# sun-huangqingbo/multiplexed-image-annotator

Hardware: AMD Instinct MI355X
Metric: cells/sec annotated (whole node) (higher is better)
Workload: dtype f16

## Files before the change

### multiplexed-image-annotator_amd/_lib.py

```python
from __future__ import annotations

import ctypes
import os
from ctypes import POINTER, c_char_p, c_double, c_float, c_int32, c_int64, c_uint32, c_uint64, c_void_p

HERE = os.path.dirname(os.path.abspath(__file__))
LIB_PATH = os.path.join(HERE, "libribca_hip.so")
if os.environ.get("RIBCA_LIB"):
    LIB_PATH = os.environ["RIBCA_LIB"] if os.path.isabs(os.environ["RIBCA_LIB"]) else os.path.join(HERE, os.environ["RIBCA_LIB"])

TEST_LIB_PATH = LIB_PATH[:-3] + "_test.so"

_lib = None
_test_lib = None

SIGNATURES = {
    "ribca_version": (c_int32, []),
    "ribca_last_error": (c_char_p, []),
    "ribca_mask_minmax": (c_int32, [c_void_p, c_int64, c_void_p, c_void_p]),
    "ribca_label_table": (c_int32, [c_void_p, c_int32, c_int32, c_int32, c_void_p, c_void_p, c_void_p]),
    "ribca_channel_min": (c_int32, [c_void_p, c_int32, c_int64, c_void_p, c_void_p]),
    "ribca_extract_patches": (c_int32, [c_void_p, c_int32, c_int32, c_int32, c_void_p, c_void_p, c_void_p, c_void_p, c_void_p, c_int32,
                                        c_void_p, c_void_p, c_void_p]),
    "ribca_extract_patches_scaled": (c_int32, [c_void_p, c_int32, c_int32, c_int32, c_void_p, c_void_p, c_void_p, c_void_p, c_void_p, c_int32,
# ... 100 lines not shown
    "ribca_test_mx_weight_bytes": (c_int64, [c_int32, c_int32, c_int32]),
    "ribca_test_mx_pack_act": (c_int32, [c_void_p, c_int32, c_int32, c_int32, c_void_p, c_void_p, c_void_p, c_void_p]),
    "ribca_test_gemm_mx_resid": (c_int32, [c_void_p, c_int32, c_void_p, c_int32, c_int32, c_int32, c_int32, c_void_p, c_void_p, c_void_p, c_void_p,
                                           c_void_p, c_void_p, c_void_p, c_int32, c_void_p, c_void_p, c_void_p, c_void_p]),
    "ribca_test_gemm_mx_resid_packed": (c_int32, [c_void_p, c_void_p, c_void_p, c_int32, c_void_p, c_void_p, c_int32, c_int32, c_void_p, c_void_p, c_int32,
                                                  c_void_p, c_void_p, c_void_p, c_void_p]),
    "ribca_test_gemm_gelu_mx": (c_int32, [c_void_p, c_int32, c_void_p, c_int32, c_int32, c_int32, c_int32, c_void_p, c_void_p, c_void_p, c_void_p,
                                          c_void_p, c_void_p, c_void_p, c_void_p]),
    "ribca_test_gemm_mx_fc1": (c_int32, [c_void_p, c_int32, c_void_p, c_int32, c_int32, c_int32, c_int32, c_void_p, c_void_p, c_void_p, c_void_p,
                                         c_void_p, c_void_p, c_void_p, c_void_p, c_void_p, c_void_p, c_void_p, c_void_p]),
    "ribca_test_qkv_attention_mx": (c_int32, [c_void_p, c_int32, c_void_p, c_int32, c_int32, c_int32, c_int32, c_void_p, c_void_p, c_void_p, c_void_p,
                                              c_void_p, c_void_p, c_void_p, c_void_p, c_void_p, c_void_p, c_void_p, c_void_p, c_int32, c_void_p]),
    "ribca_test_gemm_resid_zmx": (c_int32, [c_int32, c_void_p, c_int32, c_void_p, c_int32, c_int32, c_int32, c_int32, c_void_p, c_void_p, c_void_p,
                                            c_void_p, c_void_p, c_void_p, c_void_p, c_int32, c_void_p, c_void_p, c_void_p, c_void_p, c_void_p,
                                            c_void_p, c_int32, c_void_p]),
    "ribca_test_gemm_fold": (c_int32, [c_int32, c_void_p, c_int32, c_void_p, c_int32, c_int32, c_int32, c_int32, c_void_p, c_void_p,
                                       c_void_p, c_void_p, c_int32, c_void_p]),
    "ribca_test_qkv_attention_fold": (c_int32, [c_void_p, c_int32, c_void_p, c_int32, c_int32, c_int32, c_int32, c_void_p, c_void_p,
                                                c_void_p, c_void_p, c_void_p, c_void_p, c_void_p, c_int32, c_void_p]),
    "ribca_test_gemm_duo_gelu": (c_int32, [c_void_p, c_int32, c_void_p, c_int32, c_int32, c_int32, c_int32, c_void_p, c_void_p, c_void_p,
                                           c_void_p, c_void_p, c_int32, c_void_p]),
    "ribca_test_cell_attention": (c_int32, [c_void_p, c_int32, c_void_p, c_int32, c_int32, c_int32, c_void_p, c_void_p, c_void_p, c_void_p, c_int32,
                                            c_void_p]),
    "ribca_gemm_padded_n": (c_int32, [c_int32]),
}


class RibcaError(RuntimeError):
    pass


class _Library:

    def __init__(self, handle):
        self._handle = handle

    def __getattr__(self, name):
        if name in SIGNATURES:
            fn = getattr(self._handle, name)
        elif name in TEST_SIGNATURES:
            fn = getattr(_load_test_lib(), name)
        else:
            raise AttributeError(f"{name} is declared neither in include/ribca_hip.h nor in include/ribca_hip_test.h")
        setattr(self, name, fn)
        return fn

# ... 61 lines not shown
```

### multiplexed-image-annotator_amd/build.py

```python
from __future__ import annotations

import concurrent.futures
import os
import subprocess
import sys

HERE = os.path.dirname(os.path.abspath(__file__))
CSRC = os.path.join(HERE, "csrc")
LIB = os.path.join(HERE, "libribca_hip.so")
LIB_TEST = os.path.join(HERE, "libribca_hip_test.so")
TEST_SOURCES = ["ribca_test_api.hip"]
EXPORTS = os.path.join(CSRC, "exports.map")
SOURCES = ["gemm_split16.hip", "gemm_duo.hip", "gemm_mx.hip", "attention.hip", "cell_attention.hip", "vit_misc.hip", "preprocess.hip", "preprocess_scaled.hip", "vote.hip", "colorize.hip", "knn.hip", "umap.hip", "hdbscan.hip", "regions.hip", "spectral.hip", "scatter.hip", "celltype_stats.hip", "enrichment.hip", "autocorr.hip", "local_autocorr.hip", "cooccurrence.hip", "normalize.hip", "ribca_api.hip"]
HEADERS = ["ribca_common.h", "ribca_kernels.h", "ribca_scratch.h", "ribca_perm.h", "ribca_status.h", "ribca_internal.h", "gemm_epi.h", os.path.join("..", "..", "include", "ribca_hip.h"),
           os.path.join("..", "..", "include", "ribca_hip_test.h")]
FLAGS = ["-O3", "--offload-arch=gfx950", "-fPIC", "-std=c++17", "-Wall", "-Wno-unused-function", "-fvisibility=hidden", "-fvisibility-inlines-hidden",
         "-fno-slp-vectorize"]


def source_fingerprint() -> str:
    import hashlib
    h = hashlib.sha256()
    for name in sorted(SOURCES + TEST_SOURCES) + sorted(HEADERS):
        path = os.path.normpath(os.path.join(CSRC, name))
        h.update(os.path.basename(path).encode() + b"\0")
        with open(path, "rb") as f:
            h.update(f.read())
    h.update(" ".join(FLAGS).encode())
    return h.hexdigest()


def _hipcc() -> str:
    for cand in (os.environ.get("HIPCC"), "/opt/rocm/bin/hipcc", "hipcc"):
        if cand and (os.path.isabs(cand) and os.path.exists(cand) or not os.path.isabs(cand)):
            return cand
    raise RuntimeError("hipcc not found")
# ... 52 lines not shown
```

### multiplexed-image-annotator_amd/csrc/ribca_api.hip

```cpp
#include <hip/hip_runtime.h>

#include <cmath>
#include <cstdarg>
#include <cstdlib>
#include <cstdio>
#include <cstring>
#include <string>
#include <vector>

#include "../../include/ribca_hip.h"
#include "ribca_common.h"
#include "ribca_internal.h"
#include "ribca_kernels.h"
#include "ribca_scratch.h"
#include "ribca_status.h"

using namespace ribca;

namespace {

int fail(const std::string& msg) { return api_fail(msg.c_str()); }
int hip_fail(hipError_t e, const char* what) { return api_hip_fail(e, what); }

inline int round_up(int v, int m) { return (v + m - 1) / m * m; }
// ... 57 lines not shown
}
int api_hip_fail(hipError_t e, const char* what) { return api_fail((std::string(what) + ": " + hipGetErrorString(e)).c_str()); }
int api_finish() {
  if (!g_launch_err.empty()) {
    const std::string m = g_launch_err;
    (void)hipGetLastError();
    return api_fail(m.c_str());
  }
  const hipError_t e = hipGetLastError();
  return e == hipSuccess ? 0 : api_hip_fail(e, "kernel launch");
}
const char* api_last_error() { return g_err.c_str(); }
}

struct BlockW {
  const float *ln1w, *ln1b, *qkvb, *projb, *ln2w, *ln2b, *fc1b, *fc2b;
  const uint16_t *qkvw, *projw, *fc1w, *fc2w;
  const uint16_t* qkvwf = nullptr;
  const uint16_t* fc1wf;
  const uint16_t *projwf = nullptr, *fc2wf = nullptr;
  const float *qkvc = nullptr, *qkvb2 = nullptr, *fc1c = nullptr, *fc1b2 = nullptr;
  const uint16_t* fc2mxh = nullptr; const unsigned char* fc2mxx = nullptr;
  const uint16_t *qkvmxh = nullptr, *fc1mxh = nullptr; const unsigned char *qkvmxx = nullptr, *fc1mxx = nullptr;
};

bool env_on(const char* name) { return !(getenv(name) && atoi(getenv(name)) == 0); }
struct Switches { bool mx, mxz, cell_attn; };
const Switches& switches() {
  static const Switches sw = {env_on("RIBCA_MX"), env_on("RIBCA_MXZ"), env_on("RIBCA_CELL_ATTN")};
  return sw;
}
bool mx_on(int D) { return switches().mx && (4 * D) % 128 == 0 && gemm_mx_supported(D, 4 * D); }
bool mx_z_on(int D) { return switches().mxz && mx_on(D) && D % 192 == 0; }

struct BlockPath {
  bool fold, mx_fc2, mx_z, cell_attn;
  BlockPath precise() const { return {fold, false, false, cell_attn}; }
  bool qkv_mx3() const { return mx_z && !cell_attn; }
};
BlockPath block_path(const AttnGeom& a, bool fold) {
  return {fold, fold && mx_on(a.D), fold && mx_z_on(a.D), fold && switches().cell_attn && cell_attention_supported(a.D, a.H, a.T)};
}

struct ribca_vit {
  int D, C, K, depth, Dp;
  BlockPath path;
  char* arena = nullptr;
  size_t arena_bytes = 0;
  const float *cls, *pos, *pe_b, *norm_w, *norm_b, *head_w, *head_b;
  const float* pe_w;
  std::vector<BlockW> layers;
};

struct ribca_mae {
  int L, enc_depth, dec_depth;
  BlockPath enc_path, dec_path;
  char* arena = nullptr;
  size_t arena_bytes = 0;
  const float *cls, *pos, *pe_b, *norm_w, *norm_b, *de_b, *mask_tok, *dpos, *dnorm_w, *dnorm_b, *pred_b;
  const uint16_t *pe_w, *de_w, *pred_w;
  std::vector<BlockW> enc, dec;
};

namespace {
// ... 7 lines not shown
    L.fc1c = c.take<float>(4 * D); L.fc1b2 = c.take<float>(4 * D);
  }
  L.ln1w = c.take<float>(D); L.ln1b = c.take<float>(D);
  L.qkvb = c.take<float>(3 * D); L.projb = c.take<float>(D);
  L.ln2w = c.take<float>(D); L.ln2b = c.take<float>(D);
  L.fc1b = c.take<float>(4 * D); L.fc2b = c.take<float>(D);
  L.qkvw = c.take<uint16_t>((size_t)gemm_padded_n(3 * D) * 2 * Dp);
  if (p.fold) L.qkvwf = c.take<uint16_t>((size_t)gemm_padded_n(3 * D) * 2 * Dp);
  L.projw = c.take<uint16_t>((size_t)gemm_padded_n(D) * 2 * Dp);
  if (p.fold) L.projwf = c.take<uint16_t>((size_t)gemm_padded_n(D) * 2 * Dp);
  L.fc1w = c.take<uint16_t>((size_t)gemm_padded_n(4 * D) * 2 * Dp);
  L.fc1wf = c.take<uint16_t>((size_t)gemm_padded_n(4 * D) * 2 * Dp);
  L.fc2w = c.take<uint16_t>((size_t)gemm_padded_n(D) * 2 * H4);
  if (p.fold) L.fc2wf = c.take<uint16_t>((size_t)gemm_padded_n(D) * 2 * H4);
  if (p.mx_fc2) {
    L.fc2mxh = c.take<uint16_t>(mx_wh_bytes(round_up(D, 16), H4) / 2);
    L.fc2mxx = c.take<unsigned char>(mx_wx_bytes(round_up(D, 16), H4));
  }
  if (p.mx_z) {
    const int Kz = round_up(D, 128);
    L.qkvmxh = c.take<uint16_t>(mx_wh_bytes(3 * D, Kz) / 2); L.qkvmxx = c.take<unsigned char>(mx_wx_bytes(3 * D, Kz));
    L.fc1mxh = c.take<uint16_t>(mx_wh_bytes(4 * D, Kz) / 2); L.fc1mxx = c.take<unsigned char>(mx_wx_bytes(4 * D, Kz));
  }
}

size_t layout(ribca_vit* m, char* base) {
  Carver c(base);
  const int D = m->D;
  m->cls = c.take<float>(D);
  m->pos = c.take<float>((size_t)kTokens * D);
  m->pe_b = c.take<float>(D);
  m->pe_w = c.take<float>((size_t)D * 16 * m->C);
  m->layers.resize(m->depth);
  for (auto& L : m->layers) layout_block(c, L, D, m->path);
  m->norm_w = c.take<float>(D); m->norm_b = c.take<float>(D);
  m->head_w = c.take<float>((size_t)m->K * D); m->head_b = c.take<float>(m->K);
  return c.off;
}

size_t layout_mae(ribca_mae* m, char* base) {
  Carver c(base);
  m->cls = c.take<float>(kEncD);
  m->pos = c.take<float>((size_t)(m->L + 1) * kEncD);
  m->pe_w = c.take<uint16_t>((size_t)gemm_padded_n(kEncD) * 2 * kTokPix);
  m->pe_b = c.take<float>(kEncD);
  m->enc.resize(m->enc_depth);
// ... 30 lines not shown
  void block(const BlockW& L, int D, const BlockPath& path) {
    const int Dp = round_up(D, 32);
    copy(L.ln1w, D); copy(L.ln1b, D);
    if (path.fold) {
      pack_fold(L.qkvw, 3 * D, D, Dp, L.ln1w, L.ln1b, L.qkvc, L.qkvb2);
      launch_pack_wf(L.qkvw, 2 * Dp, gemm_padded_n(3 * D), Dp, const_cast<uint16_t*>(L.qkvwf), s);
    } else pack(L.qkvw, 3 * D, D, Dp);
    copy(L.qkvb, 3 * D);
    pack(L.projw, D, D, Dp); copy(L.projb, D);
    if (path.fold) launch_pack_wf(L.projw, 2 * Dp, gemm_padded_n(D), Dp, const_cast<uint16_t*>(L.projwf), s);
    copy(L.ln2w, D); copy(L.ln2b, D);
    if (path.fold) pack_fold(L.fc1w, 4 * D, D, Dp, L.ln2w, L.ln2b, L.fc1c, L.fc1b2);
    else pack(L.fc1w, 4 * D, D, Dp);
    copy(L.fc1b, 4 * D);
    launch_pack_wf(L.fc1w, 2 * Dp, gemm_padded_n(4 * D), Dp, const_cast<uint16_t*>(L.fc1wf), s);
    pack(L.fc2w, D, 4 * D, 4 * D); copy(L.fc2b, D);
    if (path.fold) launch_pack_wf(L.fc2w, 2 * 4 * D, gemm_padded_n(D), 4 * D, const_cast<uint16_t*>(L.fc2wf), s);
    if (path.mx_fc2) launch_mx_pack_w(L.fc2w, 2 * 4 * D, round_up(D, 16), 4 * D, 4 * D, const_cast<uint16_t*>(L.fc2mxh), const_cast<unsigned char*>(L.fc2mxx), s);
    if (path.mx_z) {
      const int Kz = round_up(D, 128);
      launch_mx_pack_w(L.qkvw, 2 * Dp, 3 * D, Dp, Kz, const_cast<uint16_t*>(L.qkvmxh), const_cast<unsigned char*>(L.qkvmxx), s);
      launch_mx_pack_w(L.fc1w, 2 * Dp, 4 * D, Dp, Kz, const_cast<uint16_t*>(L.fc1mxh), const_cast<unsigned char*>(L.fc1mxx), s);
    }
  }
};
int64_t block_params(int64_t d) { return 2 * d + 3 * d * d + 3 * d + d * d + d + 2 * d + 4 * d * d + 4 * d + 4 * d * d + d; }

struct BlockWs {
  float* z; uint16_t* xa; uint16_t* q; uint16_t* k; uint16_t* vt; uint16_t* h;
  size_t qk_bytes, vt_bytes, xa_bytes;
  uint16_t* zps = nullptr; float2* part = nullptr; float2* rs = nullptr;
  MxAct zmx = MxAct{nullptr, nullptr, nullptr, 0, 0};
  size_t zmx_rows = 0;
};
BlockWs carve_blocks(Carver& c, int cells, const AttnGeom& a, const BlockPath& p) {
  BlockWs w;
  const size_t Mc = (size_t)cells * a.T;
  const int Dp = round_up(a.D, 32);
  if (p.fold) {
    w.z = nullptr;
    w.zps = c.take<uint16_t>(Mc * 2 * Dp);
    w.part = c.take<float2>(Mc * gemm_resid_part_rows(a.D));
    w.rs = c.take<float2>(Mc);
    if (p.mx_z) {
      const int Kz = round_up(a.D, 128);
      w.zmx.hi = c.take<uint16_t>(Mc * Kz);
      w.zmx.l8 = c.take<unsigned char>(Mc * Kz);
      w.zmx.sc = c.take<unsigned char>(Mc * (Kz / 32));
      w.zmx.Kp = Kz;
      w.zmx_rows = Mc;
    }
  } else {
    w.z = c.take<float>(Mc * a.D);
  }
  w.xa_bytes = Mc * 2 * Dp * sizeof(uint16_t);
  w.xa = c.take<uint16_t>(Mc * 2 * Dp);
  const size_t qk = (size_t)cells * a.H * a.TP * 2 * a.hdq;
  w.qk_bytes = qk * sizeof(uint16_t);
  w.q = c.take<uint16_t>(qk);
  w.k = c.take<uint16_t>(qk);
  const size_t vt = attention_v_elems(a, cells);
  w.vt_bytes = vt * sizeof(uint16_t);
  w.vt = c.take<uint16_t>(vt);
  w.h = c.take<uint16_t>(Mc * 2 * 4 * a.D);
  return w;
}
int zero_pads(const BlockWs& w, const BlockPath& p, hipStream_t s) {
  HIP_TRY(hipMemsetAsync(w.xa, 0, w.xa_bytes, s));
  if (p.fold) HIP_TRY(hipMemsetAsync(w.zps, 0, w.xa_bytes, s));
  HIP_TRY(hipMemsetAsync(w.q, 0, w.qk_bytes, s));
  HIP_TRY(hipMemsetAsync(w.k, 0, w.qk_bytes, s));
  HIP_TRY(hipMemsetAsync(w.vt, 0, w.vt_bytes, s));
  if (p.mx_z) {
    HIP_TRY(hipMemsetAsync(w.zmx.hi, 0, w.zmx_rows * w.zmx.Kp * 2, s));
    HIP_TRY(hipMemsetAsync(w.zmx.l8, 0, w.zmx_rows * w.zmx.Kp, s));
    HIP_TRY(hipMemsetAsync(w.zmx.sc, 0, w.zmx_rows * (w.zmx.Kp / 32), s));
  }
  return 0;
}
void run_block(const BlockW& L, const BlockWs& w, int cells, const AttnGeom& a, hipStream_t s) {
  const int D = a.D, Dp = round_up(D, 32), ld_x = 2 * Dp, ld_h = 2 * 4 * D, Mc = cells * a.T;
  const float scale = 1.0f / sqrtf((float)a.hd);
  { ProfScope ps(P_LN, s); launch_layernorm_ps(w.z, D, L.ln1w, L.ln1b, w.xa, ld_x, Mc, D, s); }
  {
    ProfScope ps(P_QKV, s);
    GemmArgs g{w.xa, ld_x, L.qkvw, ld_x, Mc, 3 * D, Dp, L.qkvb};
    launch_gemm_qkv(g, w.q, w.k, w.vt, a, scale, s);
// ... 20 lines not shown
void resid_ps_and_stats(const GemmArgs& g, const BlockWs& w, int ldz_rows, int D, bool want_stats, int prev_stride, hipStream_t s) {
  const ResidStatGeom sg = launch_gemm_resid_ps(g, w.zps, ldz_rows, want_stats ? w.part : nullptr, w.rs, prev_stride, s);
  if (want_stats) launch_ln_finalize(w.part, sg.tiles, g.M, sg.bn, D, w.rs, s);
}
void run_block_fold(const BlockW& L, const BlockWs& w, int cells, const AttnGeom& a, const BlockPath& p, bool next_mx3, hipStream_t s) {
  const int D = a.D, Dp = round_up(D, 32), ld_x = 2 * Dp, ld_h = 2 * 4 * D, Mc = cells * a.T;
  const float scale = 1.0f / sqrtf((float)a.hd);
  MxAct zmx = w.zmx;
  zmx.M = Mc;
  if (p.cell_attn) {
    ProfScope ps(P_CELL, s);
    launch_cell_qkv_attention(w.zps, ld_x, L.qkvw, ld_x, L.qkvb2, L.qkvc, w.rs, w.xa, ld_x, cells, D, scale, s);
  } else {
    {
      ProfScope ps(P_QKV, s);
      if (p.mx_z) {
        launch_gemm_mx_qkv_ln(zmx, MxWeight{L.qkvmxh, L.qkvmxx}, Mc, 3 * D, L.qkvb2, w.rs, L.qkvc, w.q, w.k, w.vt, a, scale, s);
      } else {
        GemmArgs g{w.zps, ld_x, L.qkvw, ld_x, Mc, 3 * D, Dp, L.qkvb2, L.qkvwf};
        launch_gemm_qkv_ln(g, w.rs, L.qkvc, w.q, w.k, w.vt, a, scale, s);
      }
    }
    { ProfScope ps(P_ATTN, s); launch_attention(w.q, w.k, w.vt, w.xa, ld_x, cells, a, s); }
  }
  {
    ProfScope ps(P_PROJ, s);
    GemmArgs g{w.xa, ld_x, L.projw, ld_x, Mc, D, Dp, L.projb, L.projwf};
    if (p.mx_z) {
      const ResidStatGeom sg = launch_gemm_resid_ps(g, w.zps, ld_x, w.part, w.rs, 1, s, false, &zmx);
      launch_ln_finalize(w.part, sg.tiles, Mc, sg.bn, D, w.rs, s);
    } else {
      resid_ps_and_stats(g, w, ld_x, D, true, 1, s);
    }
  }
  if (p.mx_fc2) {
    const size_t hn = (size_t)Mc * 4 * D;
    const MxAct hmx{w.h, reinterpret_cast<unsigned char*>(w.h + hn), reinterpret_cast<unsigned char*>(w.h + hn) + hn, 4 * D, Mc};
    {
      ProfScope ps(P_FC1, s);
      if (p.mx_z) {
        launch_gemm_mx_gelu(zmx, MxWeight{L.fc1mxh, L.fc1mxx}, Mc, 4 * D, L.fc1b2, w.rs, L.fc1c, hmx, s);
      } else {
        GemmArgs g{w.zps, ld_x, L.fc1w, ld_x, Mc, 4 * D, Dp, L.fc1b2, L.fc1wf};
        (void)launch_gemm_gelu_mx(g, w.rs, L.fc1c, hmx, s);
      }
    }
// ... 555 lines not shown
```

### multiplexed-image-annotator_amd/csrc/ribca_internal.h

```cpp
#pragma once
#include <stdint.h>

#include "ribca_kernels.h"
#include "ribca_status.h"

#define RIBCA_INTERNAL_VERSION 6002

#define RIBCA_INTERNAL_FUNCS(X)                                                                                                              \
  X(api_finish) X(api_fail) X(mx_wh_bytes) X(mx_wx_bytes) X(gemm_padded_n) X(gemm_resid_bn) X(gemm_resid_tiles) X(gemm_resid_part_rows)      \
  X(gemm_mx_supported) X(cell_attention_supported) X(make_attn_geom) X(launch_pack_wf)                                                      \
  X(launch_pack_weight) X(launch_pack_weight_fold) X(launch_mx_pack_w) X(launch_mx_pack_act) X(launch_layernorm_ps) X(launch_row_stats_ps)   \
  X(launch_ln_finalize) X(launch_gemm_resid) X(launch_gemm_gelu) X(launch_gemm_qkv) X(launch_gemm_qkv_ln) X(launch_gemm_gelu_ln)             \
  X(launch_gemm_gelu_mx) X(launch_gemm_resid_ps) X(launch_gemm_mx_resid) X(launch_gemm_mx_qkv_ln) X(launch_gemm_mx_gelu) X(launch_attention) \
  X(launch_cell_qkv_attention)

namespace ribca {
struct InternalTable {
  int32_t version;
  int32_t n_funcs;
#define RIBCA_X(name) decltype(&ribca::name) name;
  RIBCA_INTERNAL_FUNCS(RIBCA_X)
#undef RIBCA_X
};
}
```

### multiplexed-image-annotator_amd/csrc/ribca_kernels.h

```cpp
#pragma once
#include <hip/hip_runtime.h>
#include <stdint.h>

namespace ribca {

int gemm_pick_bn(int N);
int gemm_padded_n(int N);

struct GemmArgs {
  const uint16_t* A; int lda;
  const uint16_t* W; int ldw;
  int M, N, Kp;
  const float* bias;
  const uint16_t* WF = nullptr;
};
void launch_pack_wf(const uint16_t* W, int ldw, int Np, int Kp, uint16_t* WF, hipStream_t s);
void launch_gemm_resid(const GemmArgs& g, float* z, int ldz, hipStream_t s);
void launch_gemm_gelu(const GemmArgs& g, uint16_t* out, int ldo, hipStream_t s);
struct ResidStatGeom { int tiles, bn; };
struct MxAct { uint16_t* hi; unsigned char* l8; unsigned char* sc; int Kp; int M; };
ResidStatGeom launch_gemm_resid_ps(const GemmArgs& g, uint16_t* z, int ldz, float2* part, const float2* prev, int prev_stride, hipStream_t s,
                                   bool force_duo = false, const MxAct* zmx = nullptr);
int gemm_resid_tiles(int N);
int gemm_resid_bn(int N);
// ... 13 lines not shown
                        int dst_per_cell, hipStream_t s);

struct MxWeight { const uint16_t* wh; const unsigned char* wx; };
size_t mx_wh_bytes(int Np, int Kp);
size_t mx_wx_bytes(int Np, int Kp);
inline size_t mx_act_hi_elems(size_t M, int Kp128) { return M * (size_t)Kp128; }
void launch_mx_pack_w(const uint16_t* W, int ldw, int Np, int Ksrc, int Kp, uint16_t* WH, unsigned char* WX, hipStream_t s);
void launch_mx_pack_act(const uint16_t* ps, int ldps, int M, int Kp, const MxAct& a, hipStream_t s);
bool gemm_mx_supported(int N, int Kp);
bool launch_gemm_gelu_mx(const GemmArgs& g, const float2* rowstat, const float* csum, const MxAct& out, hipStream_t s);
ResidStatGeom launch_gemm_mx_resid(const MxAct& A, const MxWeight& W, int M, int N, const float* bias, uint16_t* z, int ldz, float2* part,
                                   const float2* prev, int prev_stride, hipStream_t s, const MxAct* zmx = nullptr);
void launch_gemm_mx_qkv_ln(const MxAct& A, const MxWeight& W, int M, int N, const float* bias, const float2* rowstat, const float* csum, uint16_t* q,
                           uint16_t* k, uint16_t* vt, const AttnGeom& a, float scale, hipStream_t s);
void launch_gemm_mx_gelu(const MxAct& A, const MxWeight& W, int M, int N, const float* bias, const float2* rowstat, const float* csum, const MxAct& out,
                         hipStream_t s);

void launch_attention(const uint16_t* q, const uint16_t* k, const uint16_t* vt, uint16_t* out, int ldo, int cells, const AttnGeom& a,
                      hipStream_t s, int q_tiles = 0);

bool cell_attention_supported(int D, int H, int T);
void launch_cell_qkv_attention(const uint16_t* z, int ldz, const uint16_t* W, int ldw, const float* bias2, const float* csum, const float2* rowstat,
                               uint16_t* out, int ldo, int cells, int D, float scale, hipStream_t s);

void launch_layernorm_ps(const float* z, int ldz, const float* gamma, const float* beta, uint16_t* out, int ldo, int M, int D,
                         hipStream_t s);
void launch_cls_rows(float* z, int ldz, const float* cls, const float* pos, int D, int cells, int tokens_per_cell, hipStream_t s);
void launch_layernorm_gather_ps(const float* z, int ldz, const float* gamma, const float* beta, uint16_t* out, int ldo, int cells, int T,
                                int S, const int* sel, int D, hipStream_t s);
void launch_layernorm_gather_ps_from_ps(const uint16_t* z_ps, int ldz, const float* gamma, const float* beta, uint16_t* out, int ldo, int cells,
                                        int T, int S, const int* sel, int D, hipStream_t s);
void launch_rows_to_ps(const float* src, int K, uint16_t* out, int ldo, int Kp, int cells, int T, int S, const int* sel, hipStream_t s);
void launch_fill_rows(float* z, int ldz, const float* a, const float* table, int D, int cells, int T, int S, const int* sel, hipStream_t s);
void launch_pack_weight(const float* w, int N, int K, uint16_t* out, int Np, int Kp, hipStream_t s);
void launch_embed_ps(const float* patches, int c_img, const int* src_chan, int C, const float* w, const float* bias, const float* pos,
                     uint16_t* z, int ldz, int D, int cells, hipStream_t s);
void launch_cls_rows_ps(uint16_t* z, int ldz, const float* cls, const float* pos, int D, int cells, int tokens_per_cell, hipStream_t s);
void launch_head_softmax_ps(const uint16_t* z, int ldz, const float* gamma, const float* beta, const float* hw, const float* hb,
                            float* probs, int D, int K, int cells, hipStream_t s);
void launch_row_stats_ps(uint16_t* z, int ldz, int M, int D, float2* rowstat, bool recentre, hipStream_t s);
void launch_ln_finalize(const float2* part, int T, int M, int bn, int N, float2* rowstat, hipStream_t s);
void launch_pack_weight_fold(const float* w, int N, int K, const float* gamma, const float* beta, const float* bias, uint16_t* out, int Np,
                             int Kp, float* csum, float* bias2, hipStream_t s);

void launch_mask_max(const int32_t* mask, long long n, int32_t* out_max, hipStream_t s);
void launch_label_table_init(int32_t* tab_i32, unsigned long long* tab_u64, int L, hipStream_t s);
// ... 55 lines not shown
```

### multiplexed-image-annotator_amd/csrc/ribca_test_api.hip

```cpp
#include <hip/hip_runtime.h>

#include <cmath>
#include <cstdint>
#include <cstdlib>
#include <string>

#include <utility>

#include "../../include/ribca_hip.h"
#include "../../include/ribca_hip_test.h"
#include "ribca_common.h"
#include "ribca_internal.h"

using ribca::AttnGeom;
using ribca::GemmArgs;
using ribca::kHeads;
using ribca::kTokens;
using ribca::MxAct;
using ribca::MxWeight;
using ribca::ResidStatGeom;

namespace {
const ribca::InternalTable* table() {
  static const ribca::InternalTable* t = static_cast<const ribca::InternalTable*>(ribca_internal_table(RIBCA_INTERNAL_VERSION));
// ... 236 lines not shown
int ribca_test_gemm_duo_gelu(const uint16_t* A, int32_t lda, const uint16_t* W, int32_t ldw, int32_t M, int32_t N, int32_t Kp,
                             const float* bias, const float* csum, const float* rowstat, uint16_t* wf_scratch, uint16_t* out, int32_t ldo,
                             void* stream) {
  RIBCA_NEED_TABLE();
  if (M < 4096) return fail("ribca_test_gemm_duo_gelu: the forward uses this kernel for M >= 4096 only");
  if (!wf_scratch) return fail("ribca_test_gemm_duo_gelu: wf_scratch is NULL");
  if ((csum != nullptr) != (rowstat != nullptr)) return fail("ribca_test_gemm_duo_gelu: csum and rowstat go together");
  launch_pack_wf(W, ldw, gemm_padded_n(N), Kp, wf_scratch, (hipStream_t)stream);
  GemmArgs g{A, lda, W, ldw, M, N, Kp, bias, wf_scratch};
  if (csum) launch_gemm_gelu_ln(g, reinterpret_cast<const float2*>(rowstat), csum, out, ldo, (hipStream_t)stream);
  else launch_gemm_gelu(g, out, ldo, (hipStream_t)stream);
  RIBCA_FINISH();
  return 0;
}
int ribca_test_cell_attention(const uint16_t* z_ps, int32_t lda, const uint16_t* W, int32_t ldw, int32_t cells, int32_t D,
                              const float* bias2, const float* csum, const float* rowstat, uint16_t* out, int32_t ldo, void* stream) {
  RIBCA_NEED_TABLE();
  if (!cell_attention_supported(D, kHeads, kTokens)) return fail("ribca_test_cell_attention: D must be 144, 288 or 384");
  launch_cell_qkv_attention(z_ps, lda, W, ldw, bias2, csum, reinterpret_cast<const float2*>(rowstat), out, ldo, cells, D,
                            1.0f / sqrtf((float)(D / kHeads)), (hipStream_t)stream);
  RIBCA_FINISH();
  return 0;
}
int ribca_test_qkv_attention(const uint16_t* A, int32_t lda, const uint16_t* W, int32_t ldw, int32_t cells, int32_t D, int32_t Kp,
                             const float* bias, uint16_t* q, uint16_t* k, uint16_t* vt, uint16_t* out, int32_t ldo, void* stream) {
  RIBCA_NEED_TABLE();
  const AttnGeom a = make_attn_geom(D, kHeads, kTokens);
  GemmArgs g{A, lda, W, ldw, cells * kTokens, 3 * D, Kp, bias};
  launch_gemm_qkv(g, q, k, vt, a, 1.0f / sqrtf((float)a.hd), (hipStream_t)stream);
  launch_attention(q, k, vt, out, ldo, cells, a, (hipStream_t)stream, 0);
  RIBCA_FINISH();
  return 0;
}

}
```

Measured before the change: 16580.

## Fuse attention projection, LayerNorm, FC1+GELU and FC2 into one per-row MLP kernel

Adds a cell_mlp kernel for D=144 that runs the attention output projection with residual, recomputes row LayerNorm stats, then streams FC1 slices with GELU and accumulates FC2, all in registers for 64 rows per block. Weights are pre-packed into a swizzled image and streamed through a three-slot LDS ring using global_load_lds. This removes the separate proj, LN, FC1 and FC2 launches and the round trip of the 4D hidden activation through global memory. The block path enables it by default when cell attention is active, and the scratch sizes for part and h shrink accordingly. It relies on a register-heavy single kernel with a fixed shape.

```diff
diff --git a/multiplexed-image-annotator_amd/_lib.py b/multiplexed-image-annotator_amd/_lib.py
--- a/multiplexed-image-annotator_amd/_lib.py
+++ b/multiplexed-image-annotator_amd/_lib.py
@@ -146,6 +146,9 @@
                                            c_void_p, c_void_p, c_int32, c_void_p]),
     "ribca_test_cell_attention": (c_int32, [c_void_p, c_int32, c_void_p, c_int32, c_int32, c_int32, c_void_p, c_void_p, c_void_p, c_void_p, c_int32,
                                             c_void_p]),
+    "ribca_test_cell_mlp_image_bytes": (c_int64, [c_int32]),
+    "ribca_test_cell_mlp": (c_int32, [c_void_p, c_int32, c_void_p, c_void_p, c_void_p, c_void_p, c_void_p, c_void_p, c_void_p, c_void_p, c_int32,
+                                      c_void_p, c_int32, c_void_p, c_int32, c_int32, c_void_p]),
     "ribca_gemm_padded_n": (c_int32, [c_int32]),
 }
 
diff --git a/multiplexed-image-annotator_amd/build.py b/multiplexed-image-annotator_amd/build.py
--- a/multiplexed-image-annotator_amd/build.py
+++ b/multiplexed-image-annotator_amd/build.py
@@ -11,7 +11,7 @@
 LIB_TEST = os.path.join(HERE, "libribca_hip_test.so")
 TEST_SOURCES = ["ribca_test_api.hip"]
 EXPORTS = os.path.join(CSRC, "exports.map")
-SOURCES = ["gemm_split16.hip", "gemm_duo.hip", "gemm_mx.hip", "attention.hip", "cell_attention.hip", "vit_misc.hip", "preprocess.hip", "preprocess_scaled.hip", "vote.hip", "colorize.hip", "knn.hip", "umap.hip", "hdbscan.hip", "regions.hip", "spectral.hip", "scatter.hip", "celltype_stats.hip", "enrichment.hip", "autocorr.hip", "local_autocorr.hip", "cooccurrence.hip", "normalize.hip", "ribca_api.hip"]
+SOURCES = ["gemm_split16.hip", "gemm_duo.hip", "gemm_mx.hip", "attention.hip", "cell_attention.hip", "cell_mlp.hip", "vit_misc.hip", "preprocess.hip", "preprocess_scaled.hip", "vote.hip", "colorize.hip", "knn.hip", "umap.hip", "hdbscan.hip", "regions.hip", "spectral.hip", "scatter.hip", "celltype_stats.hip", "enrichment.hip", "autocorr.hip", "local_autocorr.hip", "cooccurrence.hip", "normalize.hip", "ribca_api.hip"]
 HEADERS = ["ribca_common.h", "ribca_kernels.h", "ribca_scratch.h", "ribca_perm.h", "ribca_status.h", "ribca_internal.h", "gemm_epi.h", os.path.join("..", "..", "include", "ribca_hip.h"),
            os.path.join("..", "..", "include", "ribca_hip_test.h")]
 FLAGS = ["-O3", "--offload-arch=gfx950", "-fPIC", "-std=c++17", "-Wall", "-Wno-unused-function", "-fvisibility=hidden", "-fvisibility-inlines-hidden",
diff --git a/multiplexed-image-annotator_amd/csrc/cell_mlp.hip b/multiplexed-image-annotator_amd/csrc/cell_mlp.hip
--- /dev/null
+++ b/multiplexed-image-annotator_amd/csrc/cell_mlp.hip
@@ -0,0 +1,335 @@
+
+#include "gemm_epi.h"
+#include "ribca_common.h"
+#include "ribca_kernels.h"
+
+namespace ribca {
+
+namespace {
+
+constexpr int kD = 144, kDp = 160, kH4 = 576;
+constexpr int kSlice = 96, kSlices = kH4 / kSlice;
+constexpr int kStageBig = kD * ROWB;
+constexpr int kStageFc1 = kSlice * ROWB;
+constexpr int kNkD = kDp / 32;
+constexpr int kNkS = kSlice / 32;
+constexpr int kProjBytes = kNkD * kStageBig;
+constexpr int kSliceBytes = kNkD * kStageFc1 + kNkS * kStageBig;
+constexpr int kImageBytes = kProjBytes + kSlices * kSliceBytes;
+constexpr int kRing = 3;
+constexpr int kOffC = kRing * kStageBig;
+constexpr int kOffC1 = kOffC, kOffB1 = kOffC1 + kH4 * 4, kOffBp = kOffB1 + kH4 * 4, kOffB2 = kOffBp + kD * 4;
+constexpr int kLds = kOffB2 + kD * 4;
+constexpr float kEps = 1e-6f;
+
+template <int OFF>
+__device__ __forceinline__ void lds_rd16(f16x8& dst, unsigned addr) {
+  asm volatile("ds_read_b128 %0, %1 offset:%2" : "=v"(dst) : "v"(addr), "n"(OFF) : "memory");
+}
+template <int OFF>
+__device__ __forceinline__ void lds_rd16(f32x4& dst, unsigned addr) {
+  asm volatile("ds_read_b128 %0, %1 offset:%2" : "=v"(dst) : "v"(addr), "n"(OFF) : "memory");
+}
+
+__device__ __host__ __forceinline__ int chain_col(int gq, int p) { return p < 4 ? 4 * gq + p : 16 + 4 * gq + (p - 4); }
+
+}
+
+__global__ __launch_bounds__(256) void cell_mlp_pack_kernel(const uint16_t* __restrict__ projw, const uint16_t* __restrict__ fc1w,
+                                                            const uint16_t* __restrict__ fc2w, uint16_t* __restrict__ img) {
+  const int idx = blockIdx.x * 256 + threadIdx.x;
+  if (idx >= kImageBytes / 16) return;
+  const int byte = idx * 16;
+  const uint16_t* W;
+  int ldw, nbase, s, within;
+  bool perm;
+  if (byte < kProjBytes) {
+    W = projw; ldw = 2 * kDp; nbase = 0; s = byte / kStageBig; within = byte % kStageBig; perm = false;
+  } else {
+    const int rem = byte - kProjBytes, q = rem / kSliceBytes, r2 = rem % kSliceBytes;
+    if (r2 < kNkD * kStageFc1) {
+      W = fc1w; ldw = 2 * kDp; nbase = kSlice * q; s = r2 / kStageFc1; within = r2 % kStageFc1; perm = true;
+    } else {
+      const int r3 = r2 - kNkD * kStageFc1;
+      W = fc2w; ldw = 2 * kH4; nbase = 0; s = kNkS * q + r3 / kStageBig; within = r3 % kStageBig; perm = true;
+    }
+  }
+  const int row = within / ROWB, pc = (within % ROWB) / 16;
+  const int lc = pc ^ swz_f(row), gq = lc >> 1, part = lc & 1;
+  const uint16_t* src = W + (size_t)(nbase + row) * ldw + 8 * part;
+  uint16_t v[8];
+#pragma unroll
+  for (int p = 0; p < 8; ++p) v[p] = src[ps_off(32 * s + (perm ? chain_col(gq, p) : 8 * gq + p))];
+  uint4 o;
+  o.x = v[0] | ((uint32_t)v[1] << 16); o.y = v[2] | ((uint32_t)v[3] << 16); o.z = v[4] | ((uint32_t)v[5] << 16); o.w = v[6] | ((uint32_t)v[7] << 16);
+  reinterpret_cast<uint4*>(img)[idx] = o;
+}
+
+__global__ __launch_bounds__(256, 2) void cell_mlp_kernel(const uint16_t* __restrict__ xa, int ldx, const char* __restrict__ img,
+                                                          const float* __restrict__ projb, const float* __restrict__ fc1c,
+                                                          const float* __restrict__ fc1b2, const float* __restrict__ fc2b, uint16_t* z, int ldz,
+                                                          float2* rs, int M) {
+  extern __shared__ __attribute__((aligned(16))) char smem[];
+  const int tid = threadIdx.x, lane = tid & 63;
+  const int wave = __builtin_amdgcn_readfirstlane(tid >> 6);
+  const int r16 = lane & 15, g = lane >> 4;
+  const int m = blockIdx.x * 64 + wave * 16 + r16;
+  const bool ok = m < M;
+  const int mrow = ok ? m : M - 1;
+
+  const uint16_t* xr = xa + (size_t)mrow * ldx;
+  f16x8 ahi[kNkD], alo[kNkD];
+#pragma unroll
+  for (int s = 0; s < kNkD; ++s) {
+    const uint4* p = reinterpret_cast<const uint4*>(xr + (4 * s + g) * 16);
+    ahi[s] = __builtin_bit_cast(f16x8, p[0]);
+    alo[s] = __builtin_bit_cast(f16x8, p[1]);
+  }
+  uint16_t* zr = z + (size_t)mrow * ldz;
+  uint2 zoh[kD / 16], zol[kD / 16];
+#pragma unroll
+  for (int j = 0; j < kD / 16; ++j) {
+    const uint16_t* p = zr + ps_off(16 * j + 4 * g);
+    zoh[j] = *reinterpret_cast<const uint2*>(p);
+    zol[j] = *reinterpret_cast<const uint2*>(p + 8);
+  }
+  const float pm1 = rs[mrow].y;
+  for (int i = tid; i < kH4 / 4; i += 256) {
+    reinterpret_cast<float4*>(smem + kOffC1)[i] = reinterpret_cast<const float4*>(fc1c)[i];
+    reinterpret_cast<float4*>(smem + kOffB1)[i] = reinterpret_cast<const float4*>(fc1b2)[i];
+  }
+  if (tid < kD / 4) {
+    reinterpret_cast<float4*>(smem + kOffBp)[tid] = reinterpret_cast<const float4*>(projb)[tid];
+    reinterpret_cast<float4*>(smem + kOffB2)[tid] = reinterpret_cast<const float4*>(fc2b)[tid];
+  }
+  float pm1u = pm1;
+#pragma unroll
+  for (int s = 0; s < kNkD; ++s) asm volatile("" : "+v"(ahi[s]), "+v"(alo[s]));
+#pragma unroll
+  for (int j = 0; j < kD / 16; ++j) asm volatile("" : "+v"(zoh[j].x), "+v"(zoh[j].y), "+v"(zol[j].x), "+v"(zol[j].y));
+  asm volatile("s_waitcnt vmcnt(0) lgkmcnt(0)" : "+v"(pm1u)::"memory");
+  __builtin_amdgcn_s_barrier();
+  asm volatile("" ::: "memory");
+
+  const char* gsrc = img + wave * 1024 + lane * 16;
+  auto issue = [&](auto np_c, int off, int slot) {
+    constexpr int NP = decltype(np_c)::value;
+    char* st = smem + slot * kStageBig + wave * 1024;
+#pragma unroll
+    for (int i = 0; i < (NP + 3) / 4; ++i) {
+      if (4 * i + 3 < NP || wave + 4 * i < NP)
+        __builtin_amdgcn_global_load_lds((const __attribute__((address_space(1))) void*)(gsrc + off + i * 4096),
+                                         (__attribute__((address_space(3))) void*)(st + i * 4096), 16, 0, 0);
+    }
+  };
+  constexpr std::integral_constant<int, kStageBig / 1024> kBig{};
+  constexpr std::integral_constant<int, kStageFc1 / 1024> kFc1{};
+  constexpr int kFlyBig = 4, kFlyFc1 = 3;
+
+  const unsigned lds_base = (unsigned)(uintptr_t)(__attribute__((address_space(3))) char*)smem;
+  const unsigned w_rd = lds_base + (unsigned)lds_off(r16, 2 * g);
+  const unsigned c_rd = lds_base + (unsigned)(16 * g);
+
+  auto kstep = [&](auto nt_c, int slot, const f16x8& bhi, const f16x8& blo, f32x4* acc) {
+    constexpr int NT = decltype(nt_c)::value, NG = NT / 3;
+    const unsigned ah = w_rd + (unsigned)(slot * kStageBig), al = ah ^ 16u;
+    f16x8 wh[2][3], wl[2][3];
+    lds_rd16<0>(wh[0][0], ah); lds_rd16<0>(wl[0][0], al);
+    lds_rd16<2048>(wh[0][1], ah); lds_rd16<2048>(wl[0][1], al);
+    lds_rd16<4096>(wh[0][2], ah); lds_rd16<4096>(wl[0][2], al);
+    auto group = [&](auto jb_c) {
+      constexpr int jb = decltype(jb_c)::value, cur = jb & 1, nxt = cur ^ 1;
+      if constexpr (jb + 1 < NG) {
+        lds_rd16<(3 * jb + 3) * 2048>(wh[nxt][0], ah); lds_rd16<(3 * jb + 3) * 2048>(wl[nxt][0], al);
+        lds_rd16<(3 * jb + 4) * 2048>(wh[nxt][1], ah); lds_rd16<(3 * jb + 4) * 2048>(wl[nxt][1], al);
+        lds_rd16<(3 * jb + 5) * 2048>(wh[nxt][2], ah); lds_rd16<(3 * jb + 5) * 2048>(wl[nxt][2], al);
+        asm volatile("s_waitcnt lgkmcnt(6)"
+                     : "+v"(wh[cur][0]), "+v"(wh[cur][1]), "+v"(wh[cur][2]), "+v"(wl[cur][0]), "+v"(wl[cur][1]), "+v"(wl[cur][2])::"memory");
+      } else {
+        asm volatile("s_waitcnt lgkmcnt(0)"
+                     : "+v"(wh[cur][0]), "+v"(wh[cur][1]), "+v"(wh[cur][2]), "+v"(wl[cur][0]), "+v"(wl[cur][1]), "+v"(wl[cur][2])::"memory");
+      }
+#pragma unroll
+      for (int j = 0; j < 3; ++j) acc[3 * jb + j] = mfma_f16(wl[cur][j], bhi, acc[3 * jb + j]);
+#pragma unroll
+      for (int j = 0; j < 3; ++j) acc[3 * jb + j] = mfma_f16(wh[cur][j], blo, acc[3 * jb + j]);
+#pragma unroll
+      for (int j = 0; j < 3; ++j) acc[3 * jb + j] = mfma_f16(wh[cur][j], bhi, acc[3 * jb + j]);
+    };
+    group(std::integral_constant<int, 0>{});
+    if constexpr (NG > 1) group(std::integral_constant<int, 1>{});
+    if constexpr (NG > 2) group(std::integral_constant<int, 2>{});
+  };
+  auto stage_top = [&](auto fly_c) {
+    wait_vmcnt<decltype(fly_c)::value>();
+    asm volatile("s_waitcnt lgkmcnt(0)" ::: "memory");
+    __builtin_amdgcn_s_barrier();
+    asm volatile("" ::: "memory");
+  };
+  constexpr std::integral_constant<int, kFlyBig> fBig{};
+  constexpr std::integral_constant<int, kFlyFc1> fFc1{};
+  constexpr std::integral_constant<int, 0> fNone{};
+  constexpr std::integral_constant<int, 9> t9{};
+  constexpr std::integral_constant<int, 6> t6{};
+
+  auto dsum4 = [&](double v) { v += __shfl_xor(v, 16, 64); v += __shfl_xor(v, 32, 64); return v; };
+  auto row_stats = [&](const f32x4* x, float& mean, float& rstd) {
+    double sum = 0.0;
+#pragma unroll
+    for (int j = 0; j < kD / 16; ++j) sum += ((double)x[j][0] + (double)x[j][1]) + ((double)x[j][2] + (double)x[j][3]);
+    const double md = dsum4(sum) / (double)kD;
+    double q = 0.0;
+#pragma unroll
+    for (int j = 0; j < kD / 16; ++j) {
+      const double d0 = x[j][0] - md, d1 = x[j][1] - md, d2 = x[j][2] - md, d3 = x[j][3] - md;
+      q += (d0 * d0 + d1 * d1) + (d2 * d2 + d3 * d3);
+    }
+    mean = (float)md;
+    rstd = (float)(1.0 / sqrt(dsum4(q) / (double)kD + (double)kEps));
+  };
+
+  int slot = 0;
+  issue(kBig, 0, 0);
+  issue(kBig, kStageBig, 1);
+  f32x4 acc[kD / 16];
+#pragma unroll
+  for (int j = 0; j < kD / 16; ++j) acc[j] = f32x4{0.f, 0.f, 0.f, 0.f};
+#pragma unroll
+  for (int s = 0; s < kNkD; ++s) {
+    if (s + 1 < kNkD) stage_top(fBig); else stage_top(fFc1);
+    const int nslot = slot == 0 ? 2 : slot - 1;
+    if (s + 2 < kNkD) issue(kBig, (s + 2) * kStageBig, nslot);
+    else issue(kFc1, kProjBytes + (s + 2 - kNkD) * kStageFc1, nslot);
+    kstep(t9, slot, ahi[s], alo[s], acc);
+    slot = slot == 2 ? 0 : slot + 1;
+  }
+  f16x8 zhi[kNkD], zlo[kNkD];
+  float mean2, rstd2;
+  {
+    f32x4 b4[kD / 16];
+    lds_rd16<kOffBp + 0 * 64>(b4[0], c_rd); lds_rd16<kOffBp + 1 * 64>(b4[1], c_rd); lds_rd16<kOffBp + 2 * 64>(b4[2], c_rd);
+    lds_rd16<kOffBp + 3 * 64>(b4[3], c_rd); lds_rd16<kOffBp + 4 * 64>(b4[4], c_rd); lds_rd16<kOffBp + 5 * 64>(b4[5], c_rd);
+    lds_rd16<kOffBp + 6 * 64>(b4[6], c_rd); lds_rd16<kOffBp + 7 * 64>(b4[7], c_rd); lds_rd16<kOffBp + 8 * 64>(b4[8], c_rd);
+    asm volatile("s_waitcnt lgkmcnt(0)"
+                 : "+v"(b4[0]), "+v"(b4[1]), "+v"(b4[2]), "+v"(b4[3]), "+v"(b4[4]), "+v"(b4[5]), "+v"(b4[6]), "+v"(b4[7]), "+v"(b4[8])::"memory");
+    uint2 xh[kD / 16 + 1], xl[kD / 16 + 1];
+#pragma unroll
+    for (int j = 0; j < kD / 16; ++j) {
+      const float zo[4] = {f16lo_plus_f16lo(zoh[j].x, zol[j].x), f16hi_plus_f16hi(zoh[j].x, zol[j].x), f16lo_plus_f16lo(zoh[j].y, zol[j].y),
+                           f16hi_plus_f16hi(zoh[j].y, zol[j].y)};
+      float x[4];
+#pragma unroll
+      for (int r = 0; r < 4; ++r) x[r] = clamp_f16_range((float)((double)zo[r] + ((double)acc[j][r] + ((double)b4[j][r] - (double)pm1u))));
+      acc[j] = f32x4{x[0], x[1], x[2], x[3]};
+      split4_unit(x, xh[j], xl[j]);
+    }
+    xh[kD / 16] = uint2{0u, 0u}; xl[kD / 16] = uint2{0u, 0u};
+    row_stats(acc, mean2, rstd2);
+#pragma unroll
+    for (int s = 0; s < kNkD; ++s) {
+      zhi[s] = __builtin_bit_cast(f16x8, uint4{xh[2 * s].x, xh[2 * s].y, xh[2 * s + 1].x, xh[2 * s + 1].y});
+      zlo[s] = __builtin_bit_cast(f16x8, uint4{xl[2 * s].x, xl[2 * s].y, xl[2 * s + 1].x, xl[2 * s + 1].y});
+    }
+  }
+  const float nm2 = -mean2 * rstd2;
+
+#pragma unroll
+  for (int j = 0; j < kD / 16; ++j) acc[j] = f32x4{0.f, 0.f, 0.f, 0.f};
+  for (int q = 0; q < kSlices; ++q) {
+    const int base = kProjBytes + q * kSliceBytes;
+    const bool more = q + 1 < kSlices;
+    f32x4 hacc[kSlice / 16];
+#pragma unroll
+    for (int j = 0; j < kSlice / 16; ++j) hacc[j] = f32x4{0.f, 0.f, 0.f, 0.f};
+#pragma unroll
+    for (int s = 0; s < kNkD; ++s) {
+      if (s + 1 < kNkD) stage_top(fFc1); else stage_top(fBig);
+      const int nslot = slot == 0 ? 2 : slot - 1;
+      if (s + 2 < kNkD) issue(kFc1, base + (s + 2) * kStageFc1, nslot);
+      else issue(kBig, base + kNkD * kStageFc1 + (s + 2 - kNkD) * kStageBig, nslot);
+      kstep(t6, slot, zhi[s], zlo[s], hacc);
+      slot = slot == 2 ? 0 : slot + 1;
+    }
+    f16x8 hhi[kNkS], hlo[kNkS];
+    {
+      f32x4 c4[kSlice / 16], b4[kSlice / 16];
+      const unsigned cq = c_rd + (unsigned)(q * kSlice * 4);
+      lds_rd16<kOffC1 + 0 * 64>(c4[0], cq); lds_rd16<kOffB1 + 0 * 64>(b4[0], cq);
+      lds_rd16<kOffC1 + 1 * 64>(c4[1], cq); lds_rd16<kOffB1 + 1 * 64>(b4[1], cq);
+      lds_rd16<kOffC1 + 2 * 64>(c4[2], cq); lds_rd16<kOffB1 + 2 * 64>(b4[2], cq);
+      lds_rd16<kOffC1 + 3 * 64>(c4[3], cq); lds_rd16<kOffB1 + 3 * 64>(b4[3], cq);
+      lds_rd16<kOffC1 + 4 * 64>(c4[4], cq); lds_rd16<kOffB1 + 4 * 64>(b4[4], cq);
+      lds_rd16<kOffC1 + 5 * 64>(c4[5], cq); lds_rd16<kOffB1 + 5 * 64>(b4[5], cq);
+      asm volatile("s_waitcnt lgkmcnt(0)"
+                   : "+v"(c4[0]), "+v"(c4[1]), "+v"(c4[2]), "+v"(c4[3]), "+v"(c4[4]), "+v"(c4[5]), "+v"(b4[0]), "+v"(b4[1]), "+v"(b4[2]),
+                     "+v"(b4[3]), "+v"(b4[4]), "+v"(b4[5])::"memory");
+      uint2 hh[kSlice / 16], hl[kSlice / 16];
+#pragma unroll
+      for (int j = 0; j < kSlice / 16; ++j) {
+        float x[4];
+#pragma unroll
+        for (int r = 0; r < 4; ++r) x[r] = gelu_erf1(fmaf(rstd2, hacc[j][r], fmaf(nm2, c4[j][r], b4[j][r])));
+        split4(x, hh[j], hl[j]);
+      }
+#pragma unroll
+      for (int s = 0; s < kNkS; ++s) {
+        hhi[s] = __builtin_bit_cast(f16x8, uint4{hh[2 * s].x, hh[2 * s].y, hh[2 * s + 1].x, hh[2 * s + 1].y});
+        hlo[s] = __builtin_bit_cast(f16x8, uint4{hl[2 * s].x, hl[2 * s].y, hl[2 * s + 1].x, hl[2 * s + 1].y});
+      }
+    }
+#pragma unroll
+    for (int s = 0; s < kNkS; ++s) {
+      if (s + 1 < kNkS) stage_top(fBig);
+      else if (more) stage_top(fFc1);
+      else stage_top(fNone);
+      const int nslot = slot == 0 ? 2 : slot - 1;
+      if (s + 2 < kNkS) issue(kBig, base + kNkD * kStageFc1 + (s + 2) * kStageBig, nslot);
+      else if (more) issue(kFc1, base + kSliceBytes + (s + 2 - kNkS) * kStageFc1, nslot);
+      kstep(t9, slot, hhi[s], hlo[s], acc);
+      slot = slot == 2 ? 0 : slot + 1;
+    }
+  }
+
+  {
+    f32x4 b4[kD / 16];
+    lds_rd16<kOffB2 + 0 * 64>(b4[0], c_rd); lds_rd16<kOffB2 + 1 * 64>(b4[1], c_rd); lds_rd16<kOffB2 + 2 * 64>(b4[2], c_rd);
+    lds_rd16<kOffB2 + 3 * 64>(b4[3], c_rd); lds_rd16<kOffB2 + 4 * 64>(b4[4], c_rd); lds_rd16<kOffB2 + 5 * 64>(b4[5], c_rd);
+    lds_rd16<kOffB2 + 6 * 64>(b4[6], c_rd); lds_rd16<kOffB2 + 7 * 64>(b4[7], c_rd); lds_rd16<kOffB2 + 8 * 64>(b4[8], c_rd);
+    asm volatile("s_waitcnt lgkmcnt(0)"
+                 : "+v"(b4[0]), "+v"(b4[1]), "+v"(b4[2]), "+v"(b4[3]), "+v"(b4[4]), "+v"(b4[5]), "+v"(b4[6]), "+v"(b4[7]), "+v"(b4[8])::"memory");
+#pragma unroll
+    for (int j = 0; j < kD / 16; ++j) {
+      const uint4 h = __builtin_bit_cast(uint4, zhi[j >> 1]), l = __builtin_bit_cast(uint4, zlo[j >> 1]);
+      const uint32_t h0 = (j & 1) ? h.z : h.x, h1 = (j & 1) ? h.w : h.y, l0 = (j & 1) ? l.z : l.x, l1 = (j & 1) ? l.w : l.y;
+      const float zo[4] = {f16lo_plus_f16lo(h0, l0), f16hi_plus_f16hi(h0, l0), f16lo_plus_f16lo(h1, l1), f16hi_plus_f16hi(h1, l1)};
+      float x[4];
+#pragma unroll
+      for (int r = 0; r < 4; ++r) x[r] = clamp_f16_range((float)((double)zo[r] + ((double)acc[j][r] + ((double)b4[j][r] - (double)mean2))));
+      acc[j] = f32x4{x[0], x[1], x[2], x[3]};
+      if (ok) ps_store4_pair<16>(z + (size_t)m * ldz, 16 * j + 4 * g, x);
+    }
+    float mean, rstd;
+    row_stats(acc, mean, rstd);
+    if (ok && g == 0) rs[m] = float2{rstd, mean};
+  }
+}
+
+bool cell_mlp_supported(int D) { return D == kD; }
+size_t cell_mlp_image_bytes(int D) { return D == kD ? (size_t)kImageBytes : 0; }
+
+void launch_cell_mlp_pack(const uint16_t* projw, const uint16_t* fc1w, const uint16_t* fc2w, int D, uint16_t* img, hipStream_t s) {
+  if (D != kD) { launch_error("cell_mlp: no form for D = %d", D); return; }
+  hipLaunchKernelGGL(cell_mlp_pack_kernel, dim3((kImageBytes / 16 + 255) / 256), dim3(256), 0, s, projw, fc1w, fc2w, img);
+}
+
+void launch_cell_mlp(const uint16_t* xa, int ldx, const uint16_t* img, const float* projb, const float* fc1c, const float* fc1b2, const float* fc2b,
+                     uint16_t* z, int ldz, float2* rs, int M, int D, hipStream_t s) {
+  if (M <= 0) return;
+  if (D != kD || ldx < 2 * kDp || ldz < 2 * kDp) { launch_error("cell_mlp: no form for D = %d, ldx = %d, ldz = %d", D, ldx, ldz); return; }
+  static unsigned long long attr_done = 0ull;
+  if (!ensure_dynamic_lds(reinterpret_cast<const void*>(cell_mlp_kernel), kLds, attr_done)) return;
+  hipLaunchKernelGGL(cell_mlp_kernel, dim3((M + 63) / 64), dim3(256), kLds, s, xa, ldx, reinterpret_cast<const char*>(img), projb, fc1c, fc1b2, fc2b, z,
+                     ldz, rs, M);
+}
+
+}
diff --git a/multiplexed-image-annotator_amd/csrc/ribca_api.hip b/multiplexed-image-annotator_amd/csrc/ribca_api.hip
--- a/multiplexed-image-annotator_amd/csrc/ribca_api.hip
+++ b/multiplexed-image-annotator_amd/csrc/ribca_api.hip
@@ -103,24 +103,26 @@
   const float *qkvc = nullptr, *qkvb2 = nullptr, *fc1c = nullptr, *fc1b2 = nullptr;
   const uint16_t* fc2mxh = nullptr; const unsigned char* fc2mxx = nullptr;
   const uint16_t *qkvmxh = nullptr, *fc1mxh = nullptr; const unsigned char *qkvmxx = nullptr, *fc1mxx = nullptr;
+  const uint16_t* mlpimg = nullptr;
 };
 
 bool env_on(const char* name) { return !(getenv(name) && atoi(getenv(name)) == 0); }
-struct Switches { bool mx, mxz, cell_attn; };
+struct Switches { bool mx, mxz, cell_attn, cell_mlp; };
 const Switches& switches() {
-  static const Switches sw = {env_on("RIBCA_MX"), env_on("RIBCA_MXZ"), env_on("RIBCA_CELL_ATTN")};
+  static const Switches sw = {env_on("RIBCA_MX"), env_on("RIBCA_MXZ"), env_on("RIBCA_CELL_ATTN"), env_on("RIBCA_CELL_MLP")};
   return sw;
 }
 bool mx_on(int D) { return switches().mx && (4 * D) % 128 == 0 && gemm_mx_supported(D, 4 * D); }
 bool mx_z_on(int D) { return switches().mxz && mx_on(D) && D % 192 == 0; }
 
 struct BlockPath {
-  bool fold, mx_fc2, mx_z, cell_attn;
-  BlockPath precise() const { return {fold, false, false, cell_attn}; }
+  bool fold, mx_fc2, mx_z, cell_attn, cell_mlp;
+  BlockPath precise() const { return {fold, false, false, cell_attn, cell_mlp}; }
   bool qkv_mx3() const { return mx_z && !cell_attn; }
 };
 BlockPath block_path(const AttnGeom& a, bool fold) {
-  return {fold, fold && mx_on(a.D), fold && mx_z_on(a.D), fold && switches().cell_attn && cell_attention_supported(a.D, a.H, a.T)};
+  const bool cell_attn = fold && switches().cell_attn && cell_attention_supported(a.D, a.H, a.T);
+  return {fold, fold && mx_on(a.D), fold && mx_z_on(a.D), cell_attn, cell_attn && switches().cell_mlp && cell_mlp_supported(a.D)};
 }
 
 struct ribca_vit {
@@ -174,6 +176,7 @@
     L.qkvmxh = c.take<uint16_t>(mx_wh_bytes(3 * D, Kz) / 2); L.qkvmxx = c.take<unsigned char>(mx_wx_bytes(3 * D, Kz));
     L.fc1mxh = c.take<uint16_t>(mx_wh_bytes(4 * D, Kz) / 2); L.fc1mxx = c.take<unsigned char>(mx_wx_bytes(4 * D, Kz));
   }
+  if (p.cell_mlp) L.mlpimg = c.take<uint16_t>(cell_mlp_image_bytes(D) / 2);
 }
 
 size_t layout(ribca_vit* m, char* base) {
@@ -250,6 +253,7 @@
       launch_mx_pack_w(L.qkvw, 2 * Dp, 3 * D, Dp, Kz, const_cast<uint16_t*>(L.qkvmxh), const_cast<unsigned char*>(L.qkvmxx), s);
       launch_mx_pack_w(L.fc1w, 2 * Dp, 4 * D, Dp, Kz, const_cast<uint16_t*>(L.fc1mxh), const_cast<unsigned char*>(L.fc1mxx), s);
     }
+    if (path.cell_mlp) launch_cell_mlp_pack(L.projw, L.fc1w, L.fc2w, D, const_cast<uint16_t*>(L.mlpimg), s);
   }
 };
 int64_t block_params(int64_t d) { return 2 * d + 3 * d * d + 3 * d + d * d + d + 2 * d + 4 * d * d + 4 * d + 4 * d * d + d; }
@@ -268,7 +272,7 @@
   if (p.fold) {
     w.z = nullptr;
     w.zps = c.take<uint16_t>(Mc * 2 * Dp);
-    w.part = c.take<float2>(Mc * gemm_resid_part_rows(a.D));
+    w.part = c.take<float2>((p.cell_mlp ? (size_t)cells : Mc) * gemm_resid_part_rows(a.D));
     w.rs = c.take<float2>(Mc);
     if (p.mx_z) {
       const int Kz = round_up(a.D, 128);
@@ -290,7 +294,7 @@
   const size_t vt = attention_v_elems(a, cells);
   w.vt_bytes = vt * sizeof(uint16_t);
   w.vt = c.take<uint16_t>(vt);
-  w.h = c.take<uint16_t>(Mc * 2 * 4 * a.D);
+  w.h = c.take<uint16_t>((p.cell_mlp ? (size_t)cells : Mc) * 2 * 4 * a.D);
   return w;
 }
 int zero_pads(const BlockWs& w, const BlockPath& p, hipStream_t s) {
@@ -357,6 +361,11 @@
       }
     }
     { ProfScope ps(P_ATTN, s); launch_attention(w.q, w.k, w.vt, w.xa, ld_x, cells, a, s); }
+  }
+  if (p.cell_mlp) {
+    ProfScope ps(P_FC2, s);
+    launch_cell_mlp(w.xa, ld_x, L.mlpimg, L.projb, L.fc1c, L.fc1b2, L.fc2b, w.zps, ld_x, w.rs, Mc, D, s);
+    return;
   }
   {
     ProfScope ps(P_PROJ, s);
diff --git a/multiplexed-image-annotator_amd/csrc/ribca_internal.h b/multiplexed-image-annotator_amd/csrc/ribca_internal.h
--- a/multiplexed-image-annotator_amd/csrc/ribca_internal.h
+++ b/multiplexed-image-annotator_amd/csrc/ribca_internal.h
@@ -4,7 +4,7 @@
 #include "ribca_kernels.h"
 #include "ribca_status.h"
 
-#define RIBCA_INTERNAL_VERSION 6002
+#define RIBCA_INTERNAL_VERSION 6003
 
 #define RIBCA_INTERNAL_FUNCS(X)                                                                                                              \
   X(api_finish) X(api_fail) X(mx_wh_bytes) X(mx_wx_bytes) X(gemm_padded_n) X(gemm_resid_bn) X(gemm_resid_tiles) X(gemm_resid_part_rows)      \
@@ -12,7 +12,7 @@
   X(launch_pack_weight) X(launch_pack_weight_fold) X(launch_mx_pack_w) X(launch_mx_pack_act) X(launch_layernorm_ps) X(launch_row_stats_ps)   \
   X(launch_ln_finalize) X(launch_gemm_resid) X(launch_gemm_gelu) X(launch_gemm_qkv) X(launch_gemm_qkv_ln) X(launch_gemm_gelu_ln)             \
   X(launch_gemm_gelu_mx) X(launch_gemm_resid_ps) X(launch_gemm_mx_resid) X(launch_gemm_mx_qkv_ln) X(launch_gemm_mx_gelu) X(launch_attention) \
-  X(launch_cell_qkv_attention)
+  X(launch_cell_qkv_attention) X(cell_mlp_supported) X(cell_mlp_image_bytes) X(launch_cell_mlp_pack) X(launch_cell_mlp)
 
 namespace ribca {
 struct InternalTable {
diff --git a/multiplexed-image-annotator_amd/csrc/ribca_kernels.h b/multiplexed-image-annotator_amd/csrc/ribca_kernels.h
--- a/multiplexed-image-annotator_amd/csrc/ribca_kernels.h
+++ b/multiplexed-image-annotator_amd/csrc/ribca_kernels.h
@@ -59,6 +59,12 @@
 bool cell_attention_supported(int D, int H, int T);
 void launch_cell_qkv_attention(const uint16_t* z, int ldz, const uint16_t* W, int ldw, const float* bias2, const float* csum, const float2* rowstat,
                                uint16_t* out, int ldo, int cells, int D, float scale, hipStream_t s);
+
+bool cell_mlp_supported(int D);
+size_t cell_mlp_image_bytes(int D);
+void launch_cell_mlp_pack(const uint16_t* projw, const uint16_t* fc1w, const uint16_t* fc2w, int D, uint16_t* img, hipStream_t s);
+void launch_cell_mlp(const uint16_t* xa, int ldx, const uint16_t* img, const float* projb, const float* fc1c, const float* fc1b2, const float* fc2b,
+                     uint16_t* z, int ldz, float2* rs, int M, int D, hipStream_t s);
 
 void launch_layernorm_ps(const float* z, int ldz, const float* gamma, const float* beta, uint16_t* out, int ldo, int M, int D,
                          hipStream_t s);
diff --git a/multiplexed-image-annotator_amd/csrc/ribca_test_api.hip b/multiplexed-image-annotator_amd/csrc/ribca_test_api.hip
--- a/multiplexed-image-annotator_amd/csrc/ribca_test_api.hip
+++ b/multiplexed-image-annotator_amd/csrc/ribca_test_api.hip
@@ -282,6 +282,19 @@
   RIBCA_FINISH();
   return 0;
 }
+int64_t ribca_test_cell_mlp_image_bytes(int32_t D) { if (table() == nullptr) return 0; return (int64_t)cell_mlp_image_bytes(D); }
+int ribca_test_cell_mlp(const uint16_t* xa, int32_t ldx, const uint16_t* projw, const uint16_t* fc1w, const uint16_t* fc2w, const float* projb,
+                        const float* fc1c, const float* fc1b2, const float* fc2b, uint16_t* img_scratch, int32_t pack, uint16_t* z_ps,
+                        int32_t ldz, float* rowstat, int32_t M, int32_t D, void* stream) {
+  RIBCA_NEED_TABLE();
+  if (!cell_mlp_supported(D)) return fail("ribca_test_cell_mlp: D must be 144");
+  if (!xa || !projw || !fc1w || !fc2w || !projb || !fc1c || !fc1b2 || !fc2b || !img_scratch || !z_ps || !rowstat)
+    return fail("ribca_test_cell_mlp: NULL buffer");
+  if (pack) launch_cell_mlp_pack(projw, fc1w, fc2w, D, img_scratch, (hipStream_t)stream);
+  launch_cell_mlp(xa, ldx, img_scratch, projb, fc1c, fc1b2, fc2b, z_ps, ldz, reinterpret_cast<float2*>(rowstat), M, D, (hipStream_t)stream);
+  RIBCA_FINISH();
+  return 0;
+}
 int ribca_test_qkv_attention(const uint16_t* A, int32_t lda, const uint16_t* W, int32_t ldw, int32_t cells, int32_t D, int32_t Kp,
                              const float* bias, uint16_t* q, uint16_t* k, uint16_t* vt, uint16_t* out, int32_t ldo, void* stream) {
   RIBCA_NEED_TABLE();
```

After: 16820, median of 6. +1.4%, better.
